# GANtastic3/MaskCycleGAN-VC

Measured on AMD Instinct MI355X. Metric: train iters/s (full G+D step), 80x64 mel bs=1, higher is better.
Workload: dtype f32

## Files before the change

### include/mcvc.h

```cpp
#ifndef MCVC_H
#define MCVC_H

#ifdef __cplusplus
extern "C" {
#endif

#define MCVC_ABI_VERSION 3
#define MCVC_GEN_NPARAMS 110
#define MCVC_DISC_NPARAMS 20
#define MCVC_N_MEL 80

int mcvc_version(void);

int mcvc_set_deterministic(int on);
int mcvc_get_deterministic(void);
int mcvc_set_precise(int on);
int mcvc_get_precise(void);
int mcvc_set_trunk_persistent(int on);

int mcvc_twin_begin(void);
int mcvc_twin_switch(void);
int mcvc_twin_end(void);
int mcvc_twin_launches(void);

long long mcvc_gen_packed_floats(void);
long long mcvc_disc_packed_floats(void);
long long mcvc_gen_stash_floats(int B, int T);
long long mcvc_gen_scratch_floats(int B, int T);
long long mcvc_disc_stash_floats(int B, int T);
long long mcvc_disc_scratch_floats(int B, int T);
int mcvc_gen_out_frames(int T);
int mcvc_disc_out_frames(int T);

int mcvc_gen_pack(const float* const* params, float* packed, void* stream);
int mcvc_gen_trunk_fused(int B, int T);
int mcvc_gen_pack_small_batch(const float* const* params, float* packed, int max_batch, int T, void* stream);
int mcvc_gen_pack_sets(const float* const* params, float* packed, int max_batch, int T, int sets, void* stream);
int mcvc_gen_pack_ranges(const float* const* params, float* packed, int max_batch, int T, int sets, int range_mask, void* stream);
int mcvc_disc_pack(const float* const* params, float* packed, void* stream);
int mcvc_disc_pack_small(const float* const* params, float* packed, int T, void* stream);
int mcvc_disc_pack_batch(const float* const* params, float* packed, int max_batch, int T, void* stream);

int mcvc_gen_forward(const float* const* params, const float* packed, const float* x, const float* mask,
                     float* out, float* stash, float* scratch, long long scratch_floats, int B, int T, void* stream);
int mcvc_gen_backward(const float* const* params, const float* packed, float* const* grads, const float* mask,
                      const float* dout, float* dx, int accumulate_dx, const float* stash,
                      float* scratch, long long scratch_floats, int B, int T, void* stream, void* aux_stream);
int mcvc_gen_backward_overlap(const float* const* params, const float* packed, float* const* grads, const float* mask,
                              const float* dout, float* dx, int accumulate_dx, const float* stash,
                              float* scratch, long long scratch_floats, int B, int T, void* stream, void* aux_stream,
                              void* const* milestones);

int mcvc_gen_trunk_fault(float* scratch, int B, int T, int reset, void* stream);
int mcvc_debug_trunk_fault_inject(int on);

#define MCVC_BWD_NO_JOIN 1
#define MCVC_BWD_FINE_MILESTONES 2
int mcvc_gen_backward_flags(const float* const* params, const float* packed, float* const* grads, const float* mask,
                            const float* dout, float* dx, int accumulate_dx, const float* stash,
                            float* scratch, long long scratch_floats, int B, int T, void* stream, void* aux_stream,
                            void* const* milestones, int flags);
int mcvc_gen_backward_prefix(const float* const* params, const float* packed, float* const* grads, const float* mask,
                             const float* dout, float* dx, int accumulate_dx, const float* stash, int stash_B,
                             float* scratch, long long scratch_floats, int B, int T, void* stream, void* aux_stream,
                             void* const* milestones, int flags);
int mcvc_gen_backward_window(const float* const* params, const float* packed, float* const* grads, const float* mask,
                             const float* dout, float* dx, int accumulate_dx, const float* stash, int stash_B, int stash_b0,
                             float* scratch, long long scratch_floats, int B, int T, void* stream, void* aux_stream,
                             void* const* milestones, int flags);
int mcvc_set_trunk_passes_in_flight(int n);
int mcvc_gen_trunk_persistent(int B, int T);

long long mcvc_gen_bf16_packed_bytes(void);
long long mcvc_gen_bf16_workspace_bytes(int B, int T);
int mcvc_gen_bf16_pack(const float* const* params, void* packed, void* stream);
int mcvc_gen_infer_bf16(const float* const* params, const void* packed, const float* x, const float* mask, float* out, void* workspace,
                        long long workspace_bytes, int B, int T, void* stream);

long long mcvc_bf16_conv2d_pack_bytes(int Cout, int Cin, int KH, int KW);
int mcvc_bf16_conv2d(const void* x, const float* w, const float* bias, void* y, void* wpack, int N, int H, int W, int Cin, int Cout,
                     int KH, int KW, int stride, int pad_h, int pad_w, void* stream);
long long mcvc_bf16_conv1_glu_pack_bytes(void);
int mcvc_bf16_conv1_glu(const float* x, const float* mask, const float* w, const float* b, const float* wg, const float* bg, void* y, void* wpack,
                        int B, int T, void* stream);
long long mcvc_bf16_last_conv_pack_bytes(void);
int mcvc_bf16_last_conv(const void* x, const float* w, const float* b, float* out, void* wpack, int B, int T, void* stream);
long long mcvc_bf16_c2d1d_pack_bytes(void);
int mcvc_bf16_c2d1d_norm(const void* x, const float* w, const float* gamma, const float* beta, void* y, void* wpack, int B, int W, void* stream);
long long mcvc_bf16_trunk_layer_pack_bytes(int Cin, int C, int gated);
int mcvc_bf16_trunk_layer(const void* x, const float* w, const float* w_gate, const float* gamma, const float* beta, const float* gamma_gate,
                          const float* beta_gate, const void* residual, void* y, void* wpack, int B, int W, int Cin, int C, void* stream);
int mcvc_bf16_instnorm_act(const void* x, const float* gamma, const float* beta, const float* gamma_gate, const float* beta_gate,
                           const void* residual, void* y, float* scratch, int N, int H, int W, int Cx, int act, int pixel_shuffle, void* stream);

int mcvc_disc_forward(const float* const* params, const float* packed, const float* x, float* out,
                      float* stash, float* scratch, long long scratch_floats, int B, int T, void* stream);
int mcvc_disc_backward(const float* const* params, const float* packed, float* const* grads,
                       const float* dout, int dout_is_logit_grad, float* dx, int accumulate_dx,
                       const float* stash, float* scratch, long long scratch_floats, int B, int T, void* stream,
                       void* aux_stream);
// ... 101 lines not shown
```

### maskcyclegan-vc_amd/csrc/net.hip

```cpp
#include "mcvc_common.h"
#include "twin.h"
#include "pack.h"
#include "misc.h"
#include "trunk.h"
#include "wino.h"
#include "wino4.h"
#include "sgemm.h"
#include "sampler.h"
#include "audio.h"
#include "vocoder.h"
#include "../../include/mcvc.h"
#include <string.h>
#include <algorithm>
#include <map>
#include <mutex>
#include <vector>

static int g_deterministic = [] { const char* e = getenv("MCVC_DETERMINISTIC"); return (e && atoi(e) != 0) ? 1 : 0; }();
int mcvc_deterministic() { return g_deterministic; }

namespace {

constexpr float kInEps = 1e-5f;

// ... 1978 lines not shown
        if (it != cache.end()) return it->second;
    }
    Exec ex{}; ex.dry = true;
    dry_run(ex);
    Needs n{(ex.slab_need + 3) & ~3LL, (ex.wslab_need + 3) & ~3LL, (ex.sg_need + 3) & ~3LL, (ex.sgw_need + 3) & ~3LL};
    std::lock_guard<std::mutex> lk(mu);
    cache[key] = n;
    return n;
}

static Exec make_exec(void* stream, void* aux_stream, float* scratch, long long scratch_floats, long long slab_off, const Needs& nd)
{
    Exec ex{};
    ex.s = (hipStream_t)stream; ex.s2 = (hipStream_t)aux_stream; ex.dry = false; ex.err = 0;
    ex.slabs = scratch + slab_off;
    ex.slab_cap = nd.slab;
    ex.sg = nd.sg ? scratch + slab_off + nd.slab : nullptr;
    ex.sg_cap = nd.sg;
    ex.sgw = nd.sgw ? scratch + slab_off + nd.slab + nd.sg : nullptr;
    ex.sgw_cap = nd.sgw;
    ex.wslabs = scratch + slab_off + nd.slab + nd.sg + nd.sgw;
    ex.wslab_cap = scratch_floats - slab_off - nd.slab - nd.sg - nd.sgw;
    return ex;
}

static Needs gen_needs(int B, int T)
{
    return cached_needs(1, B, T, [&](Exec& ex) {
        const GenDims d = gen_dims(B, T);
        gen_forward_impl(ex, nullptr, nullptr, nullptr, nullptr, nullptr, nullptr, d);
        float dummy = 0.f;
        gen_backward_impl(ex, nullptr, nullptr, nullptr, nullptr, nullptr, &dummy, 0, nullptr, nullptr, d);
    });
}

static Needs disc_needs(int B, int T)
{
    return cached_needs(2, B, T, [&](Exec& ex) {
        const DiscDims d = disc_dims(B, T);
        disc_forward_impl(ex, nullptr, nullptr, nullptr, nullptr, nullptr, d);
        float dummy = 0.f;
        disc_backward_impl(ex, nullptr, nullptr, nullptr, nullptr, 1, &dummy, 0, nullptr, nullptr, d);
    });
}

}

extern "C" {

int mcvc_version(void) { return MCVC_ABI_VERSION; }

static thread_local TwinCtx t_twin_ctx;
int mcvc_twin_begin(void)
{
    if (g_mcvc_twin) return MCVC_ERR_INVALID;
    t_twin_ctx.recs.clear(); t_twin_ctx.args.clear(); t_twin_ctx.next = 0; t_twin_ctx.err = 0; t_twin_ctx.phase = 1;
    g_mcvc_twin = &t_twin_ctx;
    return 0;
}
int mcvc_twin_switch(void)
{
    if (!g_mcvc_twin || g_mcvc_twin->phase != 1) return MCVC_ERR_INVALID;
    g_mcvc_twin->phase = 2;
    g_mcvc_twin->next = 0;
    return g_mcvc_twin->err;
}
int mcvc_twin_end(void)
{
    if (!g_mcvc_twin) return MCVC_ERR_INVALID;
    TwinCtx* t = g_mcvc_twin;
    g_mcvc_twin = nullptr;
    const int phase = t->phase;
    t->phase = 0;
    if (t->err) return t->err;
    if (phase != 2 || t->next != t->recs.size()) return MCVC_ERR_INVALID;
    return 0;
}
int mcvc_twin_launches(void) { return (int)t_twin_ctx.recs.size(); }

int mcvc_set_deterministic(int on) { const int was = g_deterministic; g_deterministic = on ? 1 : 0; return was; }
int mcvc_get_deterministic(void) { return g_deterministic; }
int mcvc_set_precise(int on) { const int was = g_precise; g_precise = on ? 1 : 0; return was; }
int mcvc_get_precise(void) { return g_precise; }
int mcvc_set_trunk_persistent(int on) { const int was = g_trunk_net; g_trunk_net = (on == 2) ? 2 : (on ? 1 : 0); return was; }

long long mcvc_gen_packed_floats(void) { return gen_net().packed_floats; }
long long mcvc_disc_packed_floats(void) { return disc_net().packed_floats; }
int mcvc_gen_out_frames(int T) { return gen_dims(1, T).Wu2; }
int mcvc_disc_out_frames(int T) { return disc_dims(1, T).W[3]; }

long long mcvc_gen_stash_floats(int B, int T) { return gen_stash(gen_dims(B, T)).total; }

long long mcvc_gen_scratch_floats(int B, int T)
{
    const Needs nd = gen_needs(B, T);
    return gen_scratch(gen_dims(B, T)).slabs + nd.slab + nd.sg + nd.sgw + nd.wslab + 64;
}

long long mcvc_disc_stash_floats(int B, int T)
{
    const DiscDims d = disc_dims(B, T);
    return disc_stash(d).total + (((long long)B * 80 * T + 3) & ~3LL);
}

long long mcvc_disc_scratch_floats(int B, int T)
{
    const Needs nd = disc_needs(B, T);
    return disc_scratch(disc_dims(B, T)).slabs + nd.slab + nd.sg + nd.sgw + nd.wslab + 64;
}

int mcvc_gen_pack(const float* const* params, float* packed, void* stream)
{
    int err = 0;
    const DevPackTable* t = dev_pack_table(0, [](PackTable& pt) {
        const GenNet& g = gen_net();
        const ConvSpec* all[] = {&g.conv1, &g.ds1, &g.ds2, &g.c2d1d, &g.c1d2d, &g.up1, &g.up2, &g.last};
        for (const ConvSpec* c : all) add_spec_jobs(pt, *c);
        for (int i = 0; i < 6; ++i) { add_spec_jobs(pt, g.res_vg[i]); add_spec_jobs(pt, g.res_out[i]); }
    }, &err);
    if (!t) return err;
    set_pack_skips(packed, 0);
    return pack_net(t, params, packed, (hipStream_t)stream);
}

int mcvc_gen_trunk_fused(int B, int T)
{
    if (B < 1 || T < 1 || !trunk_enabled()) return 0;
    const GenNet& g = gen_net();
    const GenDims d = gen_dims(B, T);
    const int W4 = d.W4;
    bool ok = true;
    for (int i = 0; i < 6 && ok; ++i) {
        ok = ok && mcvc_trunk_applies(g.res_vg[i].Cin, 3, g.res_vg[i].Cout, B, W4, TRUNK_IN_GLU, 1);
        ok = ok && mcvc_trunk_applies(g.res_out[i].Cin, 3, g.res_out[i].Cout, B, W4, TRUNK_IN, 1);
        ok = ok && mcvc_trunk_applies(g.res_out[i].cout_tot, 3, g.res_out[i].Cin, B, W4, TRUNK_PLAIN, 1);
        ok = ok && trunk_pick_ksplit(g.res_vg[i].cout_tot, 3, g.res_vg[i].Cin, B, W4, 0) >= 1;
    }
    ok = ok && mcvc_trunk_applies(g.c1d2d.Cin, 1, g.c1d2d.Cout, B, W4, TRUNK_IN, 1);
    ok = ok && trunk_pick_ksplit(g.c1d2d.cout_tot, 1, g.c1d2d.Cin, B, W4, 0) >= 1;
    ok = ok && trunk_pick_ksplit(g.c2d1d.Cin, 1, g.c2d1d.Cout, B, W4, 1) >= 1;
    ok = ok && mcvc_trunk_applies(g.c2d1d.cout_tot, 1, g.c2d1d.Cin, B, W4, TRUNK_PLAIN, 1);
    return ok ? 1 : 0;
}

int mcvc_gen_trunk_persistent(int B, int T)
{
    if (B < 1 || T < 1 || !trunk_enabled()) return 0;
    const int W4 = gen_dims(B, T).W4;
    int m = 0;
    if (trunk_net_enabled() && mcvc_trunk_net_applies(B, W4)) m |= 1;
    if (trunk_bwd_net_enabled() && mcvc_trunk_bwd_net_applies(B, W4)) m |= 2;
    return m;
}

int mcvc_gen_pack_sets(const float* const* params, float* packed, int max_batch, int T, int sets, void* stream)
{
    return mcvc_gen_pack_ranges(params, packed, max_batch, T, sets, 7, stream);
}

struct GenPackCfg { bool fused, wino_only, w4, w43, up1_w4, up1_w2, up2_w2; int skipped; };
static GenPackCfg gen_pack_cfg(int max_batch, int T)
{
    GenPackCfg q{};
    q.fused = true;
    for (int b = 1; b <= max_batch; ++b)
        if (!mcvc_gen_trunk_fused(b, T)) q.fused = false;
// ... 741 lines not shown
```

### maskcyclegan-vc_amd/csrc/sgemm.h

```cpp
#pragma once
#include <hip/hip_runtime.h>

struct SGemmArgs {
    const float* a; const float* a2; int k_split; long long lda;
    const float* b; long long ldb; int bseg; long long b_sn;
    float* c; float* c2; int m_split; long long ldc; int cseg; long long c_sn;
    const float* bias;
    int accumulate;
    int M, N, K;
    int nsplit; float* c_slab; long long c_split;
    int nt, mt;
};
int mcvc_sgemm_launch(const SGemmArgs& a, hipStream_t s);

struct IGemmClass { const float* a; int ntaps; long long coff; long long boff[9]; long long aoff[9]; int zs[9]; };
struct IGemmArgs {
    IGemmClass cls[4]; int ncls;
    long long a_ks; int zw;
    const float* b; long long b_cs, b_sn; int b_pitch;
    int Cb;
    int OW, P;
    float* c; long long ldc, c_sn; int c_sh, c_sw;
    const float* bias; int accumulate; int arow;
    int M, N;
    int nsplit; float* c_slab; long long c_split;
    int nt, mt, mgroup;
};
int mcvc_igemm_launch(const IGemmArgs& a, hipStream_t s);

struct WGemmArgs {
    const float* a; long long a_cs, a_sn; int a_pitch;
    const float* b; long long b_cs, b_sn; int b_pitch; long long boff[9]; int ntaps;
    int zw;
    int OW, P, NPIX;
    int M, Cin;
    float* c; float* c2; int m_split; int accumulate;
    int nsplit; float* c_slab; long long c_split;
    long long ldc; int nstages, nt, mt;
    int xcd_order;
};
int mcvc_wgemm_launch(const WGemmArgs& a, hipStream_t s);
int mcvc_wgemm_cib(int taps);

static inline int mcvc_xs_pw(int W) { return W / 2 + 4; }
static inline long long mcvc_xs_plane(int H, int W) { return (long long)(H / 2 + 1) * (W / 2 + 4); }
static inline long long mcvc_xs_floats(int C, int H, int W) { return 4LL * C * mcvc_xs_plane(H, W); }
static inline int mcvc_dyp_pitch(int OW) { return OW + 4; }
static inline long long mcvc_dyp_plane(int OH, int OW) { return (long long)(OH + 1) * (OW + 4); }

int mcvc_xs_from_dense_launch(const float* x, float* xs, int NB, int C, int H, int W, hipStream_t s);
int mcvc_dyp_from_dense_launch(const float* dy, float* dyp, int NB, int C, int OH, int OW, hipStream_t s);

int mcvc_dw_accum_launch(const float* slabs, int nslab, long long slab_stride, float* g0, float* g1, int Cout, int rows, int K9, hipStream_t s);
```

### maskcyclegan-vc_amd/csrc/sgemm_kernels.hip

```cpp
#include "sgemm.h"
#include "mcvc_common.h"
#include "trace.h"
#include "launch.h"

namespace {

typedef float f32x16 __attribute__((ext_vector_type(16)));

__device__ __forceinline__ void glds16(const float* g, float* l)
{
    __builtin_amdgcn_global_load_lds((const __attribute__((address_space(1))) void*)g, (__attribute__((address_space(3))) void*)l, 16, 0, 0);
}
__device__ __forceinline__ float zmasked(float v, unsigned m) { return __uint_as_float(__float_as_uint(v) & m); }
template <int N> __device__ __forceinline__ void wait_vm() { __builtin_amdgcn_s_waitcnt(0x0F70 | (N & 15) | ((N >> 4) << 14)); }
typedef float f32x4 __attribute__((ext_vector_type(4)));
__device__ __forceinline__ unsigned lds_addr(const float* p) { return (unsigned)(unsigned long long)(const __attribute__((address_space(3))) void*)p; }

constexpr int BM = 64, BN = 64, GK = 32, ST = 4;
constexpr int SA = GK * BM, SB = GK * BN, STAGE = SA + SB;
constexpr int NA = SA / 4 / 256, NBI = SB / 4 / 256, ND = NA + NBI;

__global__ void __launch_bounds__(256) sgemm_kernel(const Twin<SGemmArgs> tw)
{
    const SGemmArgs a = tw.v[blockIdx.z];
// ... 17 lines not shown
#pragma unroll
    for (int i = 0; i < NA; ++i) {
        const int f = tid + i * 256;
        aoff[i] = (long long)(f / (BM / 4)) * a.lda + m0 + 4 * (f % (BM / 4));
        adst[i] = (wave * 64 + i * 256) * 4;
    }
#pragma unroll
    for (int i = 0; i < NBI; ++i) {
        const int f = tid + i * 256;
        int n = n0 + 4 * (f % (BN / 4));
        if (n > a.N - 4) n = a.N - 4;
        boff[i] = (long long)(f / (BN / 4)) * a.ldb + (long long)(n / a.bseg) * a.b_sn + (n % a.bseg);
        bdst[i] = SA + (wave * 64 + i * 256) * 4;
    }
    auto issue = [&](int stage_k, int buf) {
        float* base = smem + buf * STAGE;
        const int k0 = kbase + stage_k * GK;
        const float* ab = (k0 < a.k_split) ? a.a + (long long)k0 * a.lda : a.a2 + (long long)(k0 - a.k_split) * a.lda;
        const float* bb = a.b + (long long)k0 * a.ldb;
#pragma unroll
        for (int i = 0; i < NA; ++i) glds16(ab + aoff[i], base + adst[i]);
#pragma unroll
        for (int i = 0; i < NBI; ++i) glds16(bb + boff[i], base + bdst[i]);
    };
    f32x16 acc;
#pragma unroll
    for (int r = 0; r < 16; ++r) acc[r] = 0.f;
    const int nst = Kc / GK;
#pragma unroll
    for (int s = 0; s < ST - 1; ++s)
        if (s < nst) issue(s, s);
    const int a_lane = half * BM + wm * 32 + l31;
    const int b_lane = SA + half * BN + wn * 32 + l31;
    for (int st = 0; st < nst; ++st) {
        const int newer = (nst - 1 - st) < (ST - 2) ? (nst - 1 - st) : (ST - 2);
        if (newer >= 2) wait_vm<2 * ND>(); else if (newer == 1) wait_vm<ND>(); else wait_vm<0>();
        __builtin_amdgcn_s_barrier();
        if (st + ST - 1 < nst) issue(st + ST - 1, (st + ST - 1) % ST);
        const float* sb = smem + (st % ST) * STAGE;
        float a0 = sb[a_lane], b0 = sb[b_lane];
#pragma unroll
        for (int p = 0; p < GK / 2; ++p) {
            const int q = (p + 1 < GK / 2) ? p + 1 : p;
            const float na0 = sb[a_lane + q * 2 * BM], nb0 = sb[b_lane + q * 2 * BN];
            acc = __builtin_amdgcn_mfma_f32_32x32x2f32(a0, b0, acc, 0, 0, 0);
            __builtin_amdgcn_sched_group_barrier(0x100, 2, 0);
            __builtin_amdgcn_sched_group_barrier(0x008, 1, 0);
            a0 = na0; b0 = nb0;
        }
    }
    const int n = n0 + wn * 32 + l31;
    const long long ldc = a.ldc;
    const int m_split = a.m_split, accumulate = a.accumulate;
    const float* bias = a.bias;
    float* const c1 = a.c; float* const c2 = a.c2;
    if (n < a.N) {
        const long long coff = (long long)(n / a.cseg) * a.c_sn + (n % a.cseg);
        const int mb = m0 + wm * 32 + 4 * half;
        if (ks) {
            float* slab = a.c_slab + (long long)(ks - 1) * a.c_split + (long long)mb * ldc + coff;
#pragma unroll
            for (int r = 0; r < 16; ++r) slab[(long long)((r & 3) + 8 * (r >> 2)) * ldc] = acc[r];
        } else {
            float* row0 = (mb < m_split) ? c1 + (long long)mb * ldc : c2 + (long long)(mb - m_split) * ldc;
            row0 += coff;
            float bv[16];
#pragma unroll
            for (int r = 0; r < 16; ++r) bv[r] = bias ? bias[mb + (r & 3) + 8 * (r >> 2)] : 0.f;
            if (accumulate) {
                float old[16];
#pragma unroll
                for (int r = 0; r < 16; ++r) old[r] = row0[(long long)((r & 3) + 8 * (r >> 2)) * ldc];
#pragma unroll
                for (int r = 0; r < 16; ++r) row0[(long long)((r & 3) + 8 * (r >> 2)) * ldc] = old[r] + acc[r] + bv[r];
            } else {
#pragma unroll
                for (int r = 0; r < 16; ++r) row0[(long long)((r & 3) + 8 * (r >> 2)) * ldc] = acc[r] + bv[r];
            }
        }
    }
}


template <bool AROW, bool ZFIX>
__global__ void __launch_bounds__(256) igemm_kernel(const Twin<IGemmArgs> tw)
{
    const IGemmArgs& a = tw.v[blockIdx.z];
    const IGemmClass& cl = a.cls[gridDim.y - 1 - blockIdx.y];
    extern __shared__ __attribute__((aligned(16))) float smem[];
    const int tid = threadIdx.x, lane = tid & 63;
    const int wave = __builtin_amdgcn_readfirstlane(tid >> 6);
    const int l31 = lane & 31, half = lane >> 5;
    const int wm = wave >> 1, wn = wave & 1;
    int lid;
    {
        const int total = (int)gridDim.x, linear = (int)blockIdx.x;
        const int q = total >> 3, r = total & 7, xcd = linear & 7, k = linear >> 3;
        lid = (xcd < r ? xcd * (q + 1) : r * (q + 1) + (xcd - r) * q) + k;
    }
    const int nt = a.nt, mt = a.mt, nsplit = a.nsplit, Cb = a.Cb, OW = a.OW, P = a.P, N = a.N;
    const long long a_ks = a.a_ks, b_cs = a.b_cs, b_sn = a.b_sn;
    const int b_pitch = a.b_pitch;
    const int mg = a.mgroup;
    int m_t, n_t;
    if (mg == 0) { n_t = lid % nt; lid /= nt; m_t = lid % mt; lid /= mt; }
    else {
        const int per = mt * nt;
        int r = lid % per;
        const int g = r / (mg * nt);
        const int gm = (g + 1) * mg <= mt ? mg : mt - g * mg;
        r -= g * mg * nt;
        n_t = r / gm; m_t = g * mg + r % gm;
        lid /= per;
    }
    const int n0 = n_t * BN;
    const int m0 = m_t * BM;
    const int ks = lid;
    const int Kc = cl.ntaps * Cb / nsplit;
    const int kbase = ks * Kc;
    const float* const A = cl.a;
    const float* const Bp = a.b;
    long long aoff[NA], boff[NBI]; int adst[NA], bdst[NBI];
#pragma unroll
    for (int i = 0; i < NA; ++i) {
        const int f = tid + i * 256;
        if (AROW) {
            const int row = f >> 3, pc = (f & 7) ^ ((row >> 1) & 7);
            aoff[i] = (long long)(m0 + row) * a_ks + 4 * pc;
        } else
        aoff[i] = (long long)(f / (BM / 4)) * a_ks + m0 + 4 * (f % (BM / 4));
        adst[i] = (wave * 64 + i * 256) * 4;
    }
#pragma unroll
    for (int i = 0; i < NBI; ++i) {
        const int f = tid + i * 256;
        int n = n0 + 4 * (f % (BN / 4));
        if (n > N - 4) n = N - 4;
        const int bb = n / P, rem = n - bb * P;
        const int ii = rem / OW, jj = rem - ii * OW;
        boff[i] = (long long)(f / (BN / 4)) * b_cs + (long long)bb * b_sn + (long long)ii * b_pitch + jj;
        bdst[i] = SA + (wave * 64 + i * 256) * 4;
    }
    auto issue = [&](int stage_k, int buf) {
        float* base = smem + buf * STAGE;
        const int k0 = kbase + stage_k * GK;
        const int t = k0 / Cb, c0 = k0 - t * Cb;
        const float* ab = AROW ? A + cl.aoff[t] + c0 : A + cl.aoff[t] + (long long)c0 * a_ks;
        const float* bb = Bp + cl.boff[t] + (long long)c0 * b_cs;
#pragma unroll
        for (int i = 0; i < NA; ++i) glds16(ab + aoff[i], base + adst[i]);
#pragma unroll
        for (int i = 0; i < NBI; ++i) glds16(bb + boff[i], base + bdst[i]);
    };
    f32x16 acc;
#pragma unroll
    for (int r = 0; r < 16; ++r) acc[r] = 0.f;
    const int nst = Kc / GK;
#pragma unroll
    for (int s = 0; s < ST - 1; ++s)
        if (s < nst) issue(s, s);
    const int a_lane = half * BM + wm * 32 + l31;
    const int b_lane = SA + half * BN + wn * 32 + l31;
    int zpos = 0;
    if (ZFIX) { const int w = (n0 + wn * 32 + l31) % a.zw; zpos = (w == 0) ? 1 : (w == a.zw - 1 ? 2 : 0); }
    for (int st = 0; st < nst; ++st) {
        const int newer = (nst - 1 - st) < (ST - 2) ? (nst - 1 - st) : (ST - 2);
        if (newer >= 2) wait_vm<2 * ND>(); else if (newer == 1) wait_vm<ND>(); else wait_vm<0>();
        __builtin_amdgcn_s_barrier();
        if (st + ST - 1 < nst) issue(st + ST - 1, (st + ST - 1) % ST);
        const float* sb = smem + (st % ST) * STAGE;
        unsigned zmask = 0xffffffffu;
        if (ZFIX) { const int zt = cl.zs[(kbase + st * GK) / Cb]; zmask = (zpos != 0 && zt == zpos) ? 0u : 0xffffffffu; }
        if (AROW) {
            const float* ar = sb + (wm * 32 + l31) * GK;
            const int sw = (l31 >> 1) & 7;
            const float* br = sb + SA + (16 * half) * BN + wn * 32 + l31;
            const unsigned a_addr = lds_addr(ar), b_addr = lds_addr(br);
            f32x4 av, an; float b0, b1, b2, b3, n0_, n1_, n2_, n3_;
            asm volatile("ds_read_b128 %0, %1" : "=&v"(av) : "v"(a_addr + ((((4 * half) ^ sw)) << 4)));
            asm volatile("ds_read_b32 %0, %4\n\tds_read_b32 %1, %4 offset:256\n\tds_read_b32 %2, %4 offset:512\n\tds_read_b32 %3, %4 offset:768"
                         : "=&v"(b0), "=&v"(b1), "=&v"(b2), "=&v"(b3) : "v"(b_addr));
#pragma unroll
            for (int q = 0; q < 4; ++q) {
                asm volatile("s_waitcnt lgkmcnt(0)" : "+v"(av), "+v"(b0), "+v"(b1), "+v"(b2), "+v"(b3));
                if (q < 3) {
                    asm volatile("ds_read_b128 %0, %1" : "=&v"(an) : "v"(a_addr + ((((4 * half + q + 1) ^ sw)) << 4)));
                    asm volatile("ds_read_b32 %0, %4\n\tds_read_b32 %1, %4 offset:256\n\tds_read_b32 %2, %4 offset:512\n\tds_read_b32 %3, %4 offset:768"
                                 : "=&v"(n0_), "=&v"(n1_), "=&v"(n2_), "=&v"(n3_) : "v"(b_addr + (q + 1) * 1024));
                }
                __builtin_amdgcn_sched_barrier(0);
                if (ZFIX) { b0 = zmasked(b0, zmask); b1 = zmasked(b1, zmask); b2 = zmasked(b2, zmask); b3 = zmasked(b3, zmask); }
                acc = __builtin_amdgcn_mfma_f32_32x32x2f32(av.x, b0, acc, 0, 0, 0);
                acc = __builtin_amdgcn_mfma_f32_32x32x2f32(av.y, b1, acc, 0, 0, 0);
                acc = __builtin_amdgcn_mfma_f32_32x32x2f32(av.z, b2, acc, 0, 0, 0);
                acc = __builtin_amdgcn_mfma_f32_32x32x2f32(av.w, b3, acc, 0, 0, 0);
                __builtin_amdgcn_sched_barrier(0);
                if (q < 3) { av = an; b0 = n0_; b1 = n1_; b2 = n2_; b3 = n3_; }
            }
            continue;
        }
        float a0 = sb[a_lane], b0 = sb[b_lane];
#pragma unroll
        for (int p = 0; p < GK / 2; ++p) {
            const int q = (p + 1 < GK / 2) ? p + 1 : p;
            const float na0 = sb[a_lane + q * 2 * BM], nb0 = sb[b_lane + q * 2 * BN];
            if (ZFIX) b0 = zmasked(b0, zmask);
            acc = __builtin_amdgcn_mfma_f32_32x32x2f32(a0, b0, acc, 0, 0, 0);
            __builtin_amdgcn_sched_group_barrier(0x100, 2, 0);
            __builtin_amdgcn_sched_group_barrier(0x008, 1, 0);
            a0 = na0; b0 = nb0;
        }
    }
    const int n = n0 + wn * 32 + l31;
    const long long ldc = a.ldc;
    const int accumulate = a.accumulate;
    const float* bias = a.bias;
    if (n < N) {
        const int bb = n / P, rem = n - bb * P;
        const int ii = rem / OW, jj = rem - ii * OW;
        const int mb = m0 + wm * 32 + 4 * half;
        const long long coff = cl.coff + (long long)bb * a.c_sn + (long long)ii * a.c_sh + (long long)jj * a.c_sw + (long long)mb * ldc;
        if (ks) {
            float* slab = a.c_slab + (long long)(ks - 1) * a.c_split + coff;
#pragma unroll
            for (int r = 0; r < 16; ++r) slab[(long long)((r & 3) + 8 * (r >> 2)) * ldc] = acc[r];
        } else {
            float* row0 = a.c + coff;
            float bv[16];
#pragma unroll
            for (int r = 0; r < 16; ++r) bv[r] = bias ? bias[mb + (r & 3) + 8 * (r >> 2)] : 0.f;
            if (accumulate) {
                float old[16];
#pragma unroll
                for (int r = 0; r < 16; ++r) old[r] = row0[(long long)((r & 3) + 8 * (r >> 2)) * ldc];
#pragma unroll
                for (int r = 0; r < 16; ++r) row0[(long long)((r & 3) + 8 * (r >> 2)) * ldc] = old[r] + acc[r] + bv[r];
            } else {
#pragma unroll
                for (int r = 0; r < 16; ++r) row0[(long long)((r & 3) + 8 * (r >> 2)) * ldc] = acc[r] + bv[r];
            }
        }
    }
}

struct DwAccumKArgs { const float* slabs; int nslab; long long slab_stride; float* g0; float* g1; int Cout; int rows; int K9; };
__global__ void __launch_bounds__(256) dw_accum_kernel(const Twin<DwAccumKArgs> tw)
{
    const DwAccumKArgs ka_ = tw.v[blockIdx.z];
    const float* __restrict__ slabs = ka_.slabs;
    int nslab = ka_.nslab;
    long long slab_stride = ka_.slab_stride;
    float* __restrict__ g0 = ka_.g0;
    float* __restrict__ g1 = ka_.g1;
    int Cout = ka_.Cout;
    int rows = ka_.rows;
    int K9 = ka_.K9;
    const long long i = ((long long)blockIdx.x * 256 + threadIdx.x) * 4;
    if (i >= (long long)rows * K9) return;
    float4 s = *reinterpret_cast<const float4*>(slabs + i);
    for (int k = 1; k < nslab; ++k) {
        const float4 v = *reinterpret_cast<const float4*>(slabs + (long long)k * slab_stride + i);
        s.x += v.x; s.y += v.y; s.z += v.z; s.w += v.w;
    }
    const long long split = (long long)Cout * K9;
    float4* d = reinterpret_cast<float4*>(i < split ? g0 + i : g1 + (i - split));
    float4 o = *d;
    o.x += s.x; o.y += s.y; o.z += s.z; o.w += s.w;
    *d = o;
}


struct XsConvKArgs { const float* src; float* dst; int C, H, W, pw; long long plane; int mode; };
__global__ void __launch_bounds__(256) layout_conv_kernel(const Twin<XsConvKArgs> tw)
{
    const XsConvKArgs a = tw.v[blockIdx.z];
    const long long nc = blockIdx.y;
    if (a.mode == 0) {
        const long long tot = 4 * a.plane;
        float* d = a.dst + nc * tot;
        const float* sp = a.src + nc * a.H * a.W;
        for (long long i = (long long)blockIdx.x * 256 + threadIdx.x; i < tot; i += (long long)gridDim.x * 256) {
            const int pq = (int)(i / a.plane); const int rem = (int)(i - (long long)pq * a.plane);
            const int r = rem / a.pw, c = rem - r * a.pw;
            float v = 0.f;
            if (r >= 1 && c >= 4) { const int h = 2 * (r - 1) + (pq >> 1), w = 2 * (c - 4) + (pq & 1); if (h < a.H && w < a.W) v = sp[(long long)h * a.W + w]; }
            d[i] = v;
        }
    } else {
        float* d = a.dst + nc * a.plane;
        const float* sp = a.src + nc * a.H * a.W;
        for (long long i = (long long)blockIdx.x * 256 + threadIdx.x; i < a.plane; i += (long long)gridDim.x * 256) {
            const int r = (int)(i / a.pw), c = (int)(i - (long long)r * a.pw);
            d[i] = (r < a.H && c < a.W) ? sp[(long long)r * a.W + c] : 0.f;
        }
    }
}

}

int mcvc_xs_from_dense_launch(const float* x, float* xs, int NB, int C, int H, int W, hipStream_t s)
{
    if ((H & 1) || (W & 1)) return MCVC_ERR_INVALID;
    const long long plane = mcvc_xs_plane(H, W);
    TraceScope ts(K_ELEMENTWISE, s, 0.0, 4.0 * NB * C * ((double)H * W + 4.0 * plane));
    mcvc_launch(layout_conv_kernel, dim3((unsigned)((4 * plane + 255) / 256), (unsigned)(NB * C)), dim3(256), 0, s, XsConvKArgs{x, xs, C, H, W, mcvc_xs_pw(W), plane, 0});
    return (int)hipGetLastError();
}

int mcvc_dyp_from_dense_launch(const float* dy, float* dyp, int NB, int C, int OH, int OW, hipStream_t s)
{
    const long long plane = mcvc_dyp_plane(OH, OW);
    TraceScope ts(K_ELEMENTWISE, s, 0.0, 4.0 * NB * C * ((double)OH * OW + plane));
    mcvc_launch(layout_conv_kernel, dim3((unsigned)((plane + 255) / 256), (unsigned)(NB * C)), dim3(256), 0, s, XsConvKArgs{dy, dyp, C, OH, OW, mcvc_dyp_pitch(OW), plane, 1});
    return (int)hipGetLastError();
}

int mcvc_sgemm_launch(const SGemmArgs& a0, hipStream_t s)
{
    SGemmArgs a = a0;
    if (a.nsplit < 1) a.nsplit = 1;
    if ((a.M % BM) != 0 || (a.K % (GK * a.nsplit)) != 0 || (a.N & 3) || a.N < 4 || (a.lda & 3) || (a.ldb & 3) || (a.bseg & 3) || (a.b_sn & 3) ||
        a.bseg < 4 || a.cseg < 1)
        return MCVC_ERR_INVALID;
    if (!a.a2) { a.a2 = a.a; a.k_split = a.K; }
    if (!a.c2) { a.c2 = a.c; a.m_split = a.M; }
    if (a.nsplit > 1 && !a.c_slab) return MCVC_ERR_INVALID;
    if (a.m_split & 31) return MCVC_ERR_INVALID;
    a.nt = cdiv_i(a.N, BN); a.mt = a.M / BM;
    constexpr size_t lds = (size_t)ST * STAGE * sizeof(float);
    static bool done = false;
    if (!done) {
        hipError_t e = hipFuncSetAttribute(reinterpret_cast<const void*>(sgemm_kernel), hipFuncAttributeMaxDynamicSharedMemorySize, 160 * 1024);
        if (e != hipSuccess) return (int)e;
        done = true;
    }
    TraceScope ts(K_SGEMM, s, 2.0 * a.M * a.N * a.K, 4.0 * ((double)a.K * a.M + (double)a.K * a.N + (double)a.M * a.N * a.nsplit));
    mcvc_launch(sgemm_kernel, dim3((unsigned)(a.nt * a.mt * a.nsplit)), dim3(256), lds, s, a);
    return (int)hipGetLastError();
}

int mcvc_igemm_launch(const IGemmArgs& a0, hipStream_t s)
{
    IGemmArgs a = a0;
    if (a.nsplit < 1) a.nsplit = 1;
    if (a.ncls < 1 || a.ncls > 4 || (a.M % BM) != 0 || (a.N & 3) || a.N < 4 || (a.a_ks & 3) || (a.Cb % GK) != 0 || (a.OW & 3) || a.P < a.OW || (a.P % a.OW) != 0 ||
        (a.nsplit > 1 && !a.c_slab))
        return MCVC_ERR_INVALID;
    double flops = 0.0, bytes = 0.0;
    for (int c = 0; c < a.ncls; ++c) {
        const IGemmClass& k = a.cls[c];
        if (!k.a || k.ntaps < 1 || k.ntaps > 9 || ((long long)k.ntaps * a.Cb) % (GK * a.nsplit) != 0) return MCVC_ERR_INVALID;
        const double K = (double)k.ntaps * a.Cb;
        flops += 2.0 * a.M * a.N * K;
        bytes += 4.0 * (K * a.M + (double)a.M * a.N * a.nsplit);
    }
    bytes += 4.0 * (double)a.Cb * a.N * 2.25;
    a.nt = cdiv_i(a.N, BN); a.mt = a.M / BM;
    {
        int kmax = 0;
        for (int c = 0; c < a.ncls; ++c) kmax = a.cls[c].ntaps * a.Cb > kmax ? a.cls[c].ntaps * a.Cb : kmax;
        static const int l2kb = mcvc_knob("MCVC_IGEMM_GROUP_KB", 2048);
        static const int simul = mcvc_knob("MCVC_IGEMM_GROUP_ROWS", 8);
        const long long panel = (long long)kmax * BM * 4;
        long long mg = l2kb > 0 ? (long long)l2kb * 1024 / (panel > 0 ? panel : 1) : 0;
        if (l2kb > 0 && mg < 1) mg = 1;
        if (l2kb > 0 && simul > mg && (long long)a.nt * a.mt * a.nsplit >= 8 * 64) mg = simul;
        if (mg > a.mt) mg = a.mt;
        a.mgroup = (int)mg;
    }
    constexpr size_t lds = (size_t)ST * STAGE * sizeof(float);
    static bool done = false;
    if (!done) {
        hipError_t e = hipFuncSetAttribute(reinterpret_cast<const void*>(igemm_kernel<false, false>), hipFuncAttributeMaxDynamicSharedMemorySize, 160 * 1024);
        if (e == hipSuccess) e = hipFuncSetAttribute(reinterpret_cast<const void*>(igemm_kernel<true, false>), hipFuncAttributeMaxDynamicSharedMemorySize, 160 * 1024);
        if (e == hipSuccess) e = hipFuncSetAttribute(reinterpret_cast<const void*>(igemm_kernel<false, true>), hipFuncAttributeMaxDynamicSharedMemorySize, 160 * 1024);
        if (e == hipSuccess) e = hipFuncSetAttribute(reinterpret_cast<const void*>(igemm_kernel<true, true>), hipFuncAttributeMaxDynamicSharedMemorySize, 160 * 1024);
        if (e != hipSuccess) return (int)e;
        done = true;
    }
    TraceScope ts(K_SGEMM, s, flops, bytes);
    const dim3 grid((unsigned)(a.nt * a.mt * a.nsplit), (unsigned)a.ncls);
    if (a.zw > 0) {
        if (a.arow) mcvc_launch(igemm_kernel<true, true>, grid, dim3(256), lds, s, a);
        else mcvc_launch(igemm_kernel<false, true>, grid, dim3(256), lds, s, a);
    } else {
        if (a.arow) mcvc_launch(igemm_kernel<true, false>, grid, dim3(256), lds, s, a);
        else mcvc_launch(igemm_kernel<false, false>, grid, dim3(256), lds, s, a);
    }
    return (int)hipGetLastError();
}

int mcvc_dw_accum_launch(const float* slabs, int nslab, long long slab_stride, float* g0, float* g1, int Cout, int rows, int K9, hipStream_t s)
{
    const long long n = (long long)rows * K9;
    if ((n & 3) || (((long long)Cout * K9) & 3) || (rows > Cout && !g1)) return MCVC_ERR_INVALID;
    TraceScope ts(K_ELEMENTWISE, s, 0.0, 4.0 * n * (nslab + 2.0));
    mcvc_launch(dw_accum_kernel, dim3((unsigned)((n / 4 + 255) / 256)), dim3(256), 0, s, DwAccumKArgs{slabs, nslab, slab_stride, g0, g1, Cout, rows, K9});
    return (int)hipGetLastError();
}
```

### maskcyclegan-vc_amd/mask_cyclegan_vc/_hip.py

```python
from __future__ import annotations

import ctypes
import os
from ctypes import c_float, c_int, c_longlong, c_void_p

import torch

_HERE = os.path.dirname(os.path.abspath(__file__))
LIB_PATH = os.environ.get("MCVC_LIB") or os.path.join(os.path.dirname(_HERE), "lib", "libmcvc_hip.so")

ABI_VERSION = 3
GEN_NPARAMS = 110
DISC_NPARAMS = 20
N_MEL = 80

_lib = None

_PP = ctypes.POINTER(c_void_p)

_SIGS = {
    "mcvc_version": (c_int, []),
    "mcvc_set_deterministic": (c_int, [c_int]),
    "mcvc_get_deterministic": (c_int, []),
    "mcvc_set_precise": (c_int, [c_int]),
    "mcvc_get_precise": (c_int, []),
    "mcvc_set_trunk_persistent": (c_int, [c_int]),
    "mcvc_twin_begin": (c_int, []),
    "mcvc_twin_switch": (c_int, []),
    "mcvc_twin_end": (c_int, []),
    "mcvc_twin_launches": (c_int, []),
    "mcvc_gen_packed_floats": (c_longlong, []),
    "mcvc_disc_packed_floats": (c_longlong, []),
    "mcvc_gen_stash_floats": (c_longlong, [c_int, c_int]),
    "mcvc_gen_scratch_floats": (c_longlong, [c_int, c_int]),
    "mcvc_disc_stash_floats": (c_longlong, [c_int, c_int]),
    "mcvc_disc_scratch_floats": (c_longlong, [c_int, c_int]),
    "mcvc_gen_out_frames": (c_int, [c_int]),
    "mcvc_disc_out_frames": (c_int, [c_int]),
    "mcvc_gen_pack": (c_int, [_PP, c_void_p, c_void_p]),
    "mcvc_gen_trunk_fused": (c_int, [c_int, c_int]),
    "mcvc_gen_pack_small_batch": (c_int, [_PP, c_void_p, c_int, c_int, c_void_p]),
    "mcvc_gen_pack_sets": (c_int, [_PP, c_void_p, c_int, c_int, c_int, c_void_p]),
    "mcvc_gen_pack_ranges": (c_int, [_PP, c_void_p, c_int, c_int, c_int, c_int, c_void_p]),
    "mcvc_disc_pack": (c_int, [_PP, c_void_p, c_void_p]),
    "mcvc_disc_pack_small": (c_int, [_PP, c_void_p, c_int, c_void_p]),
    "mcvc_disc_pack_batch": (c_int, [_PP, c_void_p, c_int, c_int, c_void_p]),
    "mcvc_gen_forward": (c_int, [_PP, c_void_p, c_void_p, c_void_p, c_void_p, c_void_p, c_void_p, c_longlong, c_int, c_int, c_void_p]),
    "mcvc_gen_backward": (c_int, [_PP, c_void_p, _PP, c_void_p, c_void_p, c_void_p, c_int, c_void_p, c_void_p, c_longlong, c_int, c_int, c_void_p, c_void_p]),
    "mcvc_gen_backward_overlap": (c_int, [_PP, c_void_p, _PP, c_void_p, c_void_p, c_void_p, c_int, c_void_p, c_void_p, c_longlong, c_int, c_int,
                                          c_void_p, c_void_p, _PP]),
    "mcvc_gen_backward_flags": (c_int, [_PP, c_void_p, _PP, c_void_p, c_void_p, c_void_p, c_int, c_void_p, c_void_p, c_longlong, c_int, c_int,
                                        c_void_p, c_void_p, _PP, c_int]),
    "mcvc_gen_backward_prefix": (c_int, [_PP, c_void_p, _PP, c_void_p, c_void_p, c_void_p, c_int, c_void_p, c_int, c_void_p, c_longlong, c_int, c_int,
                                         c_void_p, c_void_p, _PP, c_int]),
    "mcvc_gen_backward_window": (c_int, [_PP, c_void_p, _PP, c_void_p, c_void_p, c_void_p, c_int, c_void_p, c_int, c_int, c_void_p, c_longlong, c_int, c_int,
                                         c_void_p, c_void_p, _PP, c_int]),
    "mcvc_set_trunk_passes_in_flight": (c_int, [c_int]),
    "mcvc_gen_trunk_persistent": (c_int, [c_int, c_int]),
    "mcvc_gen_trunk_fault": (c_int, [c_void_p, c_int, c_int, c_int, c_void_p]),
    "mcvc_debug_trunk_fault_inject": (c_int, [c_int]),
    "mcvc_gen_bf16_packed_bytes": (c_longlong, []),
    "mcvc_gen_bf16_workspace_bytes": (c_longlong, [c_int, c_int]),
    "mcvc_gen_bf16_pack": (c_int, [_PP, c_void_p, c_void_p]),
    "mcvc_gen_infer_bf16": (c_int, [_PP, c_void_p, c_void_p, c_void_p, c_void_p, c_void_p, c_longlong, c_int, c_int, c_void_p]),
    "mcvc_bf16_conv2d_pack_bytes": (c_longlong, [c_int, c_int, c_int, c_int]),
    "mcvc_bf16_conv2d": (c_int, [c_void_p] * 5 + [c_int] * 10 + [c_void_p]),
    "mcvc_bf16_instnorm_act": (c_int, [c_void_p] * 8 + [c_int] * 6 + [c_void_p]),
    "mcvc_bf16_c2d1d_pack_bytes": (c_longlong, []),
    "mcvc_bf16_c2d1d_norm": (c_int, [c_void_p] * 6 + [c_int] * 2 + [c_void_p]),
    "mcvc_bf16_trunk_layer_pack_bytes": (c_longlong, [c_int] * 3),
    "mcvc_bf16_trunk_layer": (c_int, [c_void_p] * 10 + [c_int] * 4 + [c_void_p]),
    "mcvc_bf16_last_conv_pack_bytes": (c_longlong, []),
    "mcvc_bf16_last_conv": (c_int, [c_void_p] * 5 + [c_int] * 2 + [c_void_p]),
    "mcvc_bf16_conv1_glu_pack_bytes": (c_longlong, []),
    "mcvc_bf16_conv1_glu": (c_int, [c_void_p] * 8 + [c_int] * 2 + [c_void_p]),
    "mcvc_disc_forward": (c_int, [_PP, c_void_p, c_void_p, c_void_p, c_void_p, c_void_p, c_longlong, c_int, c_int, c_void_p]),
    "mcvc_disc_backward": (c_int, [_PP, c_void_p, _PP, c_void_p, c_int, c_void_p, c_int, c_void_p, c_void_p, c_longlong, c_int, c_int, c_void_p, c_void_p]),
    "mcvc_l1_loss": (c_int, [c_void_p, c_void_p, c_longlong, c_float, c_void_p, c_void_p, c_void_p, c_int, c_void_p]),
    "mcvc_lsgan_loss": (c_int, [c_void_p, c_longlong, c_float, c_float, c_void_p, c_void_p, c_void_p, c_void_p]),
    "mcvc_loss_combine": (c_int, [c_void_p, c_int, c_void_p, c_void_p, c_void_p, c_void_p]),
    "mcvc_adam_step": (c_int, [c_void_p, c_void_p, c_void_p, c_void_p, c_longlong, c_float, c_float, c_float, c_float, c_int, c_float, c_void_p]),
    "mcvc_adam_step2": (c_int, [c_void_p, c_void_p, c_void_p, c_int, c_void_p, c_void_p, c_longlong, c_float, c_float, c_float, c_float, c_int, c_float, c_void_p]),
    "mcvc_gen_update_ranges": (c_int, [_PP, c_void_p, c_void_p, c_int, c_int, c_int, c_void_p, c_void_p, c_void_p, c_void_p, c_void_p,
                                       c_float, c_float, c_float, c_float, c_int, c_float, c_int, c_void_p]),
    "mcvc_disc_update_batch": (c_int, [_PP, c_void_p, c_void_p, c_int, c_int, c_void_p, c_void_p, c_void_p, c_void_p, c_void_p,
                                       c_float, c_float, c_float, c_float, c_int, c_float, c_int, c_void_p]),
    "mcvc_draw_batch": (c_int, [c_void_p, c_void_p, c_int, c_longlong, c_void_p, c_void_p, c_int, c_longlong, c_int, c_int, c_int,
                                ctypes.c_ulonglong, ctypes.c_ulonglong, c_void_p, c_void_p, c_void_p, c_void_p, c_void_p, c_void_p]),
    "mcvc_audio_frames": (c_int, [c_int]),
    "mcvc_audio_basis_floats": (c_longlong, []),
    "mcvc_audio_basis_init": (c_int, [c_void_p]),
    "mcvc_audio_plan": (c_int, [c_void_p, c_int, c_void_p, c_void_p, c_int, ctypes.POINTER(c_int)]),
    "mcvc_audio_log_mel": (c_int, [c_void_p, c_longlong, c_void_p, c_int, c_void_p, c_void_p, c_longlong, c_void_p]),
    "mcvc_voc_out_samples": (c_int, [c_int]),
    "mcvc_voc_launches": (c_int, []),
    "mcvc_voc_packed_floats": (c_longlong, []),
    "mcvc_voc_pack": (c_int, [_PP, c_void_p]),
    "mcvc_voc_workspace_floats": (c_longlong, [c_int, c_int]),
    "mcvc_voc_decode": (c_int, [c_void_p, c_void_p, c_void_p, c_void_p, c_longlong, c_int, c_int, c_void_p]),
    "mcvc_voc_layer_packed_floats": (c_longlong, [c_int] * 5),
    "mcvc_voc_layer_pack": (c_int, [c_int] + [c_void_p] * 5 + [c_int] * 4),
    "mcvc_voc_layer": (c_int, [c_int] + [c_void_p] * 4 + [c_int] * 8 + [c_void_p]),
    "mcvc_axpy": (c_int, [c_void_p, c_void_p, c_float, c_longlong, c_void_p]),
    "mcvc_conv2d_pack_floats": (c_longlong, [c_int, c_int, c_int, c_int]),
    "mcvc_conv2d_forward": (c_int, [c_void_p] * 6 + [c_int] * 12 + [c_void_p]),
    "mcvc_conv2d_dgrad": (c_int, [c_void_p] * 5 + [c_int] * 11 + [c_void_p]),
    "mcvc_conv2d_wgrad_slab_floats": (c_longlong, [c_int] * 10),
    "mcvc_conv2d_wgrad": (c_int, [c_void_p] * 4 + [c_longlong] + [c_int] * 10 + [c_void_p]),
# ... 90 lines not shown
```

Baseline: 178.1.

## Add smaller igemm tile variants chosen when the 64x64 grid is undersized

Templates the implicit-GEMM kernel on tile size (64x64, 64x32, 32x32) with matching wave count, LDS staging and B-read offsets. When the 64x64 workgroup count falls below a threshold and there is no zero-fix path, the launcher picks a smaller tile. The goal is to fill more CUs on the small bs=1 convolutions. The cost is less operand reuse per tile and extra template instantiations; the choice can be overridden by a knob or API setter.

```diff
diff --git a/include/mcvc.h b/include/mcvc.h
--- a/include/mcvc.h
+++ b/include/mcvc.h
@@ -16,6 +16,8 @@
 int mcvc_get_deterministic(void);
 int mcvc_set_precise(int on);
 int mcvc_get_precise(void);
+int mcvc_set_igemm_tile(int form);
+int mcvc_get_igemm_plan(int* form, int* nsplit);
 int mcvc_set_trunk_persistent(int on);
 
 int mcvc_twin_begin(void);
diff --git a/maskcyclegan-vc_amd/csrc/net.hip b/maskcyclegan-vc_amd/csrc/net.hip
--- a/maskcyclegan-vc_amd/csrc/net.hip
+++ b/maskcyclegan-vc_amd/csrc/net.hip
@@ -2084,6 +2084,8 @@
 int mcvc_get_deterministic(void) { return g_deterministic; }
 int mcvc_set_precise(int on) { const int was = g_precise; g_precise = on ? 1 : 0; return was; }
 int mcvc_get_precise(void) { return g_precise; }
+int mcvc_set_igemm_tile(int form) { return mcvc_igemm_tile_set(form); }
+int mcvc_get_igemm_plan(int* form, int* nsplit) { mcvc_igemm_last_plan(form, nsplit); return 0; }
 int mcvc_set_trunk_persistent(int on) { const int was = g_trunk_net; g_trunk_net = (on == 2) ? 2 : (on ? 1 : 0); return was; }
 
 long long mcvc_gen_packed_floats(void) { return gen_net().packed_floats; }
diff --git a/maskcyclegan-vc_amd/csrc/sgemm.h b/maskcyclegan-vc_amd/csrc/sgemm.h
--- a/maskcyclegan-vc_amd/csrc/sgemm.h
+++ b/maskcyclegan-vc_amd/csrc/sgemm.h
@@ -27,6 +27,8 @@
     int nt, mt, mgroup;
 };
 int mcvc_igemm_launch(const IGemmArgs& a, hipStream_t s);
+int mcvc_igemm_tile_set(int form);
+void mcvc_igemm_last_plan(int* form, int* nsplit);
 
 struct WGemmArgs {
     const float* a; long long a_cs, a_sn; int a_pitch;
diff --git a/maskcyclegan-vc_amd/csrc/sgemm_kernels.hip b/maskcyclegan-vc_amd/csrc/sgemm_kernels.hip
--- a/maskcyclegan-vc_amd/csrc/sgemm_kernels.hip
+++ b/maskcyclegan-vc_amd/csrc/sgemm_kernels.hip
@@ -123,16 +123,26 @@
 }
 
 
-template <bool AROW, bool ZFIX>
-__global__ void __launch_bounds__(256) igemm_kernel(const Twin<IGemmArgs> tw)
-{
+template <int TM, int TN> struct IgTile {
+    static constexpr int WAVES = (TM / 32) * (TN / 32), THREADS = 64 * WAVES;
+    static constexpr int SA = GK * TM, SB = GK * TN, STAGE = SA + SB;
+    static constexpr int NA = SA / 4 / THREADS, NBI = SB / 4 / THREADS, ND = NA + NBI;
+    static constexpr size_t LDS = (size_t)ST * STAGE * sizeof(float);
+    static_assert(TM % 32 == 0 && TN % 32 == 0 && SA % (4 * THREADS) == 0 && SB % (4 * THREADS) == 0, "whole 16-byte pieces per lane and stage");
+    static_assert(2 * ND <= 63, "two stages of LDS-DMA in flight must fit the 6-bit vmcnt");
+};
+template <int TM, int TN, bool AROW, bool ZFIX>
+__global__ void __launch_bounds__(64 * (TM / 32) * (TN / 32)) igemm_kernel(const Twin<IGemmArgs> tw)
+{
+    typedef IgTile<TM, TN> T;
+    constexpr int BM = TM, BN = TN, THREADS = T::THREADS, SA = T::SA, STAGE = T::STAGE, NA = T::NA, NBI = T::NBI, ND = T::ND;
     const IGemmArgs& a = tw.v[blockIdx.z];
     const IGemmClass& cl = a.cls[gridDim.y - 1 - blockIdx.y];
     extern __shared__ __attribute__((aligned(16))) float smem[];
     const int tid = threadIdx.x, lane = tid & 63;
     const int wave = __builtin_amdgcn_readfirstlane(tid >> 6);
     const int l31 = lane & 31, half = lane >> 5;
-    const int wm = wave >> 1, wn = wave & 1;
+    const int wm = wave / (BN / 32), wn = wave % (BN / 32);
     int lid;
     {
         const int total = (int)gridDim.x, linear = (int)blockIdx.x;
@@ -164,23 +174,23 @@
     long long aoff[NA], boff[NBI]; int adst[NA], bdst[NBI];
 #pragma unroll
     for (int i = 0; i < NA; ++i) {
-        const int f = tid + i * 256;
+        const int f = tid + i * THREADS;
         if (AROW) {
             const int row = f >> 3, pc = (f & 7) ^ ((row >> 1) & 7);
             aoff[i] = (long long)(m0 + row) * a_ks + 4 * pc;
         } else
         aoff[i] = (long long)(f / (BM / 4)) * a_ks + m0 + 4 * (f % (BM / 4));
-        adst[i] = (wave * 64 + i * 256) * 4;
+        adst[i] = (wave * 64 + i * THREADS) * 4;
     }
 #pragma unroll
     for (int i = 0; i < NBI; ++i) {
-        const int f = tid + i * 256;
+        const int f = tid + i * THREADS;
         int n = n0 + 4 * (f % (BN / 4));
         if (n > N - 4) n = N - 4;
         const int bb = n / P, rem = n - bb * P;
         const int ii = rem / OW, jj = rem - ii * OW;
         boff[i] = (long long)(f / (BN / 4)) * b_cs + (long long)bb * b_sn + (long long)ii * b_pitch + jj;
-        bdst[i] = SA + (wave * 64 + i * 256) * 4;
+        bdst[i] = SA + (wave * 64 + i * THREADS) * 4;
     }
     auto issue = [&](int stage_k, int buf) {
         float* base = smem + buf * STAGE;
@@ -219,15 +229,15 @@
             const unsigned a_addr = lds_addr(ar), b_addr = lds_addr(br);
             f32x4 av, an; float b0, b1, b2, b3, n0_, n1_, n2_, n3_;
             asm volatile("ds_read_b128 %0, %1" : "=&v"(av) : "v"(a_addr + ((((4 * half) ^ sw)) << 4)));
-            asm volatile("ds_read_b32 %0, %4\n\tds_read_b32 %1, %4 offset:256\n\tds_read_b32 %2, %4 offset:512\n\tds_read_b32 %3, %4 offset:768"
-                         : "=&v"(b0), "=&v"(b1), "=&v"(b2), "=&v"(b3) : "v"(b_addr));
+            asm volatile("ds_read_b32 %0, %4\n\tds_read_b32 %1, %4 offset:%5\n\tds_read_b32 %2, %4 offset:%6\n\tds_read_b32 %3, %4 offset:%7"
+                         : "=&v"(b0), "=&v"(b1), "=&v"(b2), "=&v"(b3) : "v"(b_addr), "n"(BN * 4), "n"(BN * 8), "n"(BN * 12));
 #pragma unroll
             for (int q = 0; q < 4; ++q) {
                 asm volatile("s_waitcnt lgkmcnt(0)" : "+v"(av), "+v"(b0), "+v"(b1), "+v"(b2), "+v"(b3));
                 if (q < 3) {
                     asm volatile("ds_read_b128 %0, %1" : "=&v"(an) : "v"(a_addr + ((((4 * half + q + 1) ^ sw)) << 4)));
-                    asm volatile("ds_read_b32 %0, %4\n\tds_read_b32 %1, %4 offset:256\n\tds_read_b32 %2, %4 offset:512\n\tds_read_b32 %3, %4 offset:768"
-                                 : "=&v"(n0_), "=&v"(n1_), "=&v"(n2_), "=&v"(n3_) : "v"(b_addr + (q + 1) * 1024));
+                    asm volatile("ds_read_b32 %0, %4\n\tds_read_b32 %1, %4 offset:%5\n\tds_read_b32 %2, %4 offset:%6\n\tds_read_b32 %3, %4 offset:%7"
+                                 : "=&v"(n0_), "=&v"(n1_), "=&v"(n2_), "=&v"(n3_) : "v"(b_addr + (q + 1) * (BN * 16)), "n"(BN * 4), "n"(BN * 8), "n"(BN * 12));
                 }
                 __builtin_amdgcn_sched_barrier(0);
                 if (ZFIX) { b0 = zmasked(b0, zmask); b1 = zmasked(b1, zmask); b2 = zmasked(b2, zmask); b3 = zmasked(b3, zmask); }
@@ -380,11 +390,57 @@
     return (int)hipGetLastError();
 }
 
+static int g_igemm_tile = 0;
+static thread_local int t_igemm_form = 0, t_igemm_nsplit = 0;
+int mcvc_igemm_tile_set(int form) { const int was = g_igemm_tile; g_igemm_tile = (form >= 1 && form <= 3) ? form : 0; return was; }
+void mcvc_igemm_last_plan(int* form, int* nsplit) { if (form) *form = t_igemm_form; if (nsplit) *nsplit = t_igemm_nsplit; }
+
+template <int TM, int TN>
+static int igemm_launch_tile(IGemmArgs& a, hipStream_t s)
+{
+    typedef IgTile<TM, TN> T;
+    a.nt = cdiv_i(a.N, TN); a.mt = a.M / TM;
+    {
+        int kmax = 0;
+        for (int c = 0; c < a.ncls; ++c) kmax = a.cls[c].ntaps * a.Cb > kmax ? a.cls[c].ntaps * a.Cb : kmax;
+        static const int l2kb = mcvc_knob("MCVC_IGEMM_GROUP_KB", 2048);
+        static const int simul = mcvc_knob("MCVC_IGEMM_GROUP_ROWS", 8);
+        const long long panel = (long long)kmax * TM * 4;
+        long long mg = l2kb > 0 ? (long long)l2kb * 1024 / (panel > 0 ? panel : 1) : 0;
+        if (l2kb > 0 && mg < 1) mg = 1;
+        if (l2kb > 0 && simul > mg && (long long)cdiv_i(a.N, 64) * (a.M / 64) * a.nsplit >= 8 * 64) mg = simul;
+        if (mg > a.mt) mg = a.mt;
+        a.mgroup = (int)mg;
+    }
+    static bool done = false;
+    if (!done) {
+        hipError_t e = hipFuncSetAttribute(reinterpret_cast<const void*>(igemm_kernel<TM, TN, false, false>), hipFuncAttributeMaxDynamicSharedMemorySize, 160 * 1024);
+        if (e == hipSuccess) e = hipFuncSetAttribute(reinterpret_cast<const void*>(igemm_kernel<TM, TN, true, false>), hipFuncAttributeMaxDynamicSharedMemorySize, 160 * 1024);
+        if (TM == 64 && TN == 64) {
+            if (e == hipSuccess) e = hipFuncSetAttribute(reinterpret_cast<const void*>(igemm_kernel<64, 64, false, true>), hipFuncAttributeMaxDynamicSharedMemorySize, 160 * 1024);
+            if (e == hipSuccess) e = hipFuncSetAttribute(reinterpret_cast<const void*>(igemm_kernel<64, 64, true, true>), hipFuncAttributeMaxDynamicSharedMemorySize, 160 * 1024);
+        }
+        if (e != hipSuccess) return (int)e;
+        done = true;
+    }
+    const dim3 grid((unsigned)(a.nt * a.mt * a.nsplit), (unsigned)a.ncls);
+    if constexpr (TM == 64 && TN == 64) {
+        if (a.zw > 0) {
+            if (a.arow) mcvc_launch(igemm_kernel<64, 64, true, true>, grid, dim3(T::THREADS), T::LDS, s, a);
+            else mcvc_launch(igemm_kernel<64, 64, false, true>, grid, dim3(T::THREADS), T::LDS, s, a);
+            return (int)hipGetLastError();
+        }
+    }
+    if (a.arow) mcvc_launch(igemm_kernel<TM, TN, true, false>, grid, dim3(T::THREADS), T::LDS, s, a);
+    else mcvc_launch(igemm_kernel<TM, TN, false, false>, grid, dim3(T::THREADS), T::LDS, s, a);
+    return (int)hipGetLastError();
+}
+
 int mcvc_igemm_launch(const IGemmArgs& a0, hipStream_t s)
 {
     IGemmArgs a = a0;
     if (a.nsplit < 1) a.nsplit = 1;
-    if (a.ncls < 1 || a.ncls > 4 || (a.M % BM) != 0 || (a.N & 3) || a.N < 4 || (a.a_ks & 3) || (a.Cb % GK) != 0 || (a.OW & 3) || a.P < a.OW || (a.P % a.OW) != 0 ||
+    if (a.ncls < 1 || a.ncls > 4 || (a.M % 64) != 0 || (a.N & 3) || a.N < 4 || (a.a_ks & 3) || (a.Cb % GK) != 0 || (a.OW & 3) || a.P < a.OW || (a.P % a.OW) != 0 ||
         (a.nsplit > 1 && !a.c_slab))
         return MCVC_ERR_INVALID;
     double flops = 0.0, bytes = 0.0;
@@ -396,39 +452,20 @@
         bytes += 4.0 * (K * a.M + (double)a.M * a.N * a.nsplit);
     }
     bytes += 4.0 * (double)a.Cb * a.N * 2.25;
-    a.nt = cdiv_i(a.N, BN); a.mt = a.M / BM;
-    {
-        int kmax = 0;
-        for (int c = 0; c < a.ncls; ++c) kmax = a.cls[c].ntaps * a.Cb > kmax ? a.cls[c].ntaps * a.Cb : kmax;
-        static const int l2kb = mcvc_knob("MCVC_IGEMM_GROUP_KB", 2048);
-        static const int simul = mcvc_knob("MCVC_IGEMM_GROUP_ROWS", 8);
-        const long long panel = (long long)kmax * BM * 4;
-        long long mg = l2kb > 0 ? (long long)l2kb * 1024 / (panel > 0 ? panel : 1) : 0;
-        if (l2kb > 0 && mg < 1) mg = 1;
-        if (l2kb > 0 && simul > mg && (long long)a.nt * a.mt * a.nsplit >= 8 * 64) mg = simul;
-        if (mg > a.mt) mg = a.mt;
-        a.mgroup = (int)mg;
-    }
-    constexpr size_t lds = (size_t)ST * STAGE * sizeof(float);
-    static bool done = false;
-    if (!done) {
-        hipError_t e = hipFuncSetAttribute(reinterpret_cast<const void*>(igemm_kernel<false, false>), hipFuncAttributeMaxDynamicSharedMemorySize, 160 * 1024);
-        if (e == hipSuccess) e = hipFuncSetAttribute(reinterpret_cast<const void*>(igemm_kernel<true, false>), hipFuncAttributeMaxDynamicSharedMemorySize, 160 * 1024);
-        if (e == hipSuccess) e = hipFuncSetAttribute(reinterpret_cast<const void*>(igemm_kernel<false, true>), hipFuncAttributeMaxDynamicSharedMemorySize, 160 * 1024);
-        if (e == hipSuccess) e = hipFuncSetAttribute(reinterpret_cast<const void*>(igemm_kernel<true, true>), hipFuncAttributeMaxDynamicSharedMemorySize, 160 * 1024);
-        if (e != hipSuccess) return (int)e;
-        done = true;
-    }
+    int form = 1;
+    if (a.zw == 0) {
+        static const int forced = mcvc_knob("MCVC_IGEMM_TILE", 0);
+        static const int small_wgs = mcvc_knob("MCVC_IGEMM_TILE_WGS", 512);
+        static const int small_form = mcvc_knob("MCVC_IGEMM_TILE_SMALL", 3);
+        const long long wg64 = (long long)cdiv_i(a.N, 64) * (a.M / 64) * a.nsplit * a.ncls;
+        form = g_igemm_tile ? g_igemm_tile : (forced >= 1 && forced <= 3) ? forced : (wg64 < small_wgs ? small_form : 1);
+        if (form < 1 || form > 3) form = 1;
+    }
+    t_igemm_form = form; t_igemm_nsplit = a.nsplit;
     TraceScope ts(K_SGEMM, s, flops, bytes);
-    const dim3 grid((unsigned)(a.nt * a.mt * a.nsplit), (unsigned)a.ncls);
-    if (a.zw > 0) {
-        if (a.arow) mcvc_launch(igemm_kernel<true, true>, grid, dim3(256), lds, s, a);
-        else mcvc_launch(igemm_kernel<false, true>, grid, dim3(256), lds, s, a);
-    } else {
-        if (a.arow) mcvc_launch(igemm_kernel<true, false>, grid, dim3(256), lds, s, a);
-        else mcvc_launch(igemm_kernel<false, false>, grid, dim3(256), lds, s, a);
-    }
-    return (int)hipGetLastError();
+    if (form == 3) return igemm_launch_tile<32, 32>(a, s);
+    if (form == 2) return igemm_launch_tile<64, 32>(a, s);
+    return igemm_launch_tile<64, 64>(a, s);
 }
 
 int mcvc_dw_accum_launch(const float* slabs, int nslab, long long slab_stride, float* g0, float* g1, int Cout, int rows, int K9, hipStream_t s)
diff --git a/maskcyclegan-vc_amd/mask_cyclegan_vc/_hip.py b/maskcyclegan-vc_amd/mask_cyclegan_vc/_hip.py
--- a/maskcyclegan-vc_amd/mask_cyclegan_vc/_hip.py
+++ b/maskcyclegan-vc_amd/mask_cyclegan_vc/_hip.py
@@ -24,6 +24,8 @@
     "mcvc_get_deterministic": (c_int, []),
     "mcvc_set_precise": (c_int, [c_int]),
     "mcvc_get_precise": (c_int, []),
+    "mcvc_set_igemm_tile": (c_int, [c_int]),
+    "mcvc_get_igemm_plan": (c_int, [ctypes.POINTER(c_int), ctypes.POINTER(c_int)]),
     "mcvc_set_trunk_persistent": (c_int, [c_int]),
     "mcvc_twin_begin": (c_int, []),
     "mcvc_twin_switch": (c_int, []),
```

Result: slower. 169.9 (-4.6%).
